# Levicoz/Options-model

Hardware: AMD Instinct MI355X
Metric: paths x steps / sec (whole American pricing: path-gen + LSM + mean) (higher is better)
Workload: dtype f32

## Files before the change

### options_model_amd/_build.py

```python
from __future__ import annotations

import os
import shutil
import subprocess
import sys

_HERE = os.path.dirname(os.path.abspath(__file__))
CSRC = os.path.join(_HERE, "csrc")
LIBDIR = os.path.join(_HERE, "lib")
LIB = os.path.join(LIBDIR, "libomc.so")
SOURCES = ["omc_paths.hip", "omc_lsm.hip", "omc_batch.hip", "omc_mlp.hip", "omc_mlp_batch.hip", "omc_mlp_apply.hip", "omc_nn_epoch.hip", "omc_contnet.hip", "omc_rows.hip", "omc_ols7.hip", "omc_greeks.hip", "omc_barrier.hip", "omc_dividend.hip", "omc_jump.hip", "omc_basket.hip", "omc_bounds.hip", "omc_basket_bounds.hip", "omc_runnerup_bounds.hip", "omc_heston_bounds.hip", "omc_heston_sv_bounds.hip", "omc_basket_greeks.hip", "omc_chain.hip", "omc_comm.hip", "omc_p2p.hip",
           "omc_api.hip", "omc_api_price.hip", "omc_api_seq.hip", "omc_api_batch.hip", "omc_api_nn.hip",
           "omc_api_bounds.hip", "omc_api_chain.hip", "omc_api_dividend.hip", "omc_api_jump.hip", "omc_api_basket.hip",
           "omc_api_basket_bounds.hip", "omc_api_runnerup_bounds.hip", "omc_api_basket_greeks.hip",
           "omc_api_heston_bounds.hip"]
HEADERS = ["omc_ctx.h", "omc_device.h", "omc_dispatch.h", "omc_crit.h", "omc_kernels.h", "omc_lsm_dev.h", "omc_paths_dev.h", "omc_contnet_dev.h", "omc_mlp_dev.h", "omc_mlp_quad_dev.h", "omc_batch.h", "omc_greeks.h", "omc_barrier.h", "omc_dividend.h", "omc_jump.h", "omc_basket.h", "omc_basket_dev.h", "omc_bounds.h", "omc_bounds_dev.h", "omc_bounds2_dev.h", "omc_basket_bounds.h", "omc_runnerup_bounds.h", "omc_heston_bounds.h", "omc_heston_sv_bounds.h", "omc_basket_greeks.h", "omc_chain.h", "omc_comm.h", "omc_p2p.h",
           os.path.join("..", "..", "include", "omc.h")]
ARCH = "gfx950"
FLAGS_STAMP = os.path.join(LIBDIR, "libomc.flags")


def _flags() -> str:
    return " ".join(os.environ.get("OMC_HIPCC_FLAGS", "").split())


def _hipcc() -> str:
    for cand in (os.environ.get("HIPCC"), shutil.which("hipcc"), "/opt/rocm/bin/hipcc"):
        if cand and os.path.exists(cand):
            return cand
    raise RuntimeError("hipcc not found: libomc.so cannot be built (ROCm toolchain required)")


def _stale() -> bool:
    if not os.path.exists(LIB):
        return True
    try:
        built_with = open(FLAGS_STAMP).read().strip()
    except OSError:
        built_with = ""
    if built_with != _flags():
        return True
    t = os.path.getmtime(LIB)
    deps = [os.path.join(CSRC, s) for s in SOURCES + HEADERS] + [os.path.abspath(__file__)]
    return any(os.path.getmtime(d) > t for d in deps)


def build(force: bool = False, verbose: bool = False) -> str:
    if not force and not _stale():
        return LIB
# ... 32 lines not shown
```

### options_model_amd/csrc/omc_api.hip

```cpp
#include <sched.h>

#include "omc_ctx.h"

namespace omc::abi {

thread_local std::string g_err;
size_t g_alloc_limit = 0;

int check_market(double S0, double K, double T, double r)
{
    if (!(S0 > 0) || !(K > 0) || !(T > 0)) return fail(-1, "S0, K, T must be positive.");
    if (!(r >= 0)) return fail(-2, "r must be non-negative.");
    return 0;
}

int check_sizes(int64_t n_paths, int n_steps)
{
    if (n_paths <= 0 || n_steps <= 0)
        return fail(-3, "num_simulations and num_time_steps must be positive integers.");
    if (n_steps > omc::kMaxSteps) return fail(-8, "num_time_steps exceeds the supported maximum (4094).");
    return 0;
}

int check_matrix(const void* S, int64_t ld, int64_t n_paths)
// ... 679 lines not shown
    int rc = bind_in(c);
    if (rc) return rc;
    if (!bytes) return 0;
    HIP_TRY(hipMemcpyAsync(dst, src, bytes, kind, c->stream));
    HIP_TRY(hipStreamSynchronize(c->stream));
    return 0;
}

int omc_memcpy_h2d(omc_ctx* c, void* dst, const void* src, size_t bytes)
{
    return copy_and_wait(c, dst, src, bytes, hipMemcpyHostToDevice);
}

int omc_memcpy_d2h(omc_ctx* c, void* dst, const void* src, size_t bytes)
{
    return copy_and_wait(c, dst, src, bytes, hipMemcpyDeviceToHost);
}

int omc_set_option(omc_ctx* c, const char* key, int64_t value)
{
    if (!c || !key) return fail(-7, "null pointer.");
    if (!strcmp(key, "gbm_vec")) c->gbm_vec = (int)value;
    else if (!strcmp(key, "alloc_limit")) g_alloc_limit = value > 0 ? (size_t)value : 0;
    else if (!strcmp(key, "fold_antithetic")) c->fold = value <= 0 ? 0 : (value >= 2 ? 2 : 1);
    else if (!strcmp(key, "pass2_tables")) c->pass2_tables = value ? 1 : 0;
    else if (!strcmp(key, "pass2_tables_irregular_every")) c->pass2_irr_every = value > 0 ? (int)value : 0;
    else if (!strcmp(key, "heston_vec")) c->heston_vec = (int)value;
    else if (!strcmp(key, "world_size")) c->world = value > 0 ? (int)value : 1;
    else if (!strcmp(key, "step_graph")) c->step_graph = value < 0 ? -1 : (value ? 1 : 0);
    else if (!strcmp(key, "seq_overlap")) c->seq_overlap = value < 0 ? -1 : (value ? 1 : 0);
    else if (!strcmp(key, "seq_event_stride")) c->seq_event_stride = value > 0 ? (int)value : 0;
    else if (!strcmp(key, "seq_step_k")) c->seq_step_k = value < 0 ? -1 : (int)(value > 32 ? 32 : value);
    else if (!strcmp(key, "seq_two_pass_k")) c->seq_two_pass_k = value < 0 ? -1 : (int)(value > 32 ? 32 : value);
    else if (!strcmp(key, "chain_fused")) c->chain_fused = value ? 1 : 0;
    else if (!strcmp(key, "chain_k")) c->chain_k = value < 1 ? -1 : (int)(value > 16 ? 16 : value);
    else if (!strcmp(key, "seq_step_wgs")) c->seq_step_wgs = value > 0 ? (int)value : 0;
    else if (!strcmp(key, "p2p_exchange")) c->p2p_use = value ? 1 : 0;
    else if (!strcmp(key, "p2p_deadline_ms") || !strcmp(key, "p2p_first_deadline_ms")) {
        if (value <= 0) return fail(-4, "a p2p deadline must be positive.");
        (key[4] == 'f' ? c->p2p_first_deadline_s : c->p2p_deadline_s) = (double)value * 1e-3;
        if (c->p2p) omc::p2p_set_deadline(c->p2p, c->p2p_deadline_s, c->p2p_first_deadline_s);
    }
    else return fail(-4, "unknown option key.");
    return 0;
}

int omc_set_allreduce_hook(omc_ctx* c, omc_allreduce_fn fn, void* user)
{
    if (!c) return fail(-7, "null context.");
    if (fn) {
        int rc;
        if ((rc = bind(c))) return rc;
        if ((rc = c->seq_vote.ensure(kVoteBytes))) return rc;
    }
    c->hook = fn;
    c->hook_user = user;
    return 0;
}

int omc_comm_unique_id(void* uid_out, size_t bytes)
{
    if (!uid_out || bytes < (size_t)omc::kCommUidBytes) return fail(-7, "unique-id buffer must hold 128 bytes.");
    std::string err;
    const int rc = omc::comm_unique_id(uid_out, &err);
    if (rc) return fail(rc, err.c_str());
    return 0;
// ... 116 lines not shown
```

### options_model_amd/csrc/omc_api_seq.hip

```cpp
#include <cstdlib>

#include "omc_ctx.h"

using namespace omc::abi;

extern "C" {

static int pricing_events(omc_ctx* c, int i, hipEvent_t** out)
{
    const int k = c->seq_event_stride, s = i == 0 ? 0 : (k > 0 && i % k == 0) ? i / k : -1;
    *out = s == 0 ? c->ev : nullptr;
    if (s <= 0) return 0;
    while (c->ev_pool.size() < 7 * (size_t)s) {
        hipEvent_t e = nullptr;
        HIP_TRY(hipEventCreate(&e));
        c->ev_pool.push_back(e);
    }
    *out = c->ev_pool.data() + 7 * (size_t)(s - 1);
    return 0;
}

static bool seq_overlap_enabled(const omc_ctx* c)
{
    if (c->seq_overlap >= 0) return c->seq_overlap != 0;
// ... 295 lines not shown
            q.T != p[0].T)
            break;
        double c0q, gq;
        omc::gbm_fold_constants(q.S0, q.K, q.r, q.sigma, q.T, q.n_steps, &c0q, &gq);
        if (c0q != c0 || gq != g) break;
    }
    return run;
}

static size_t seq_group_matrix_bytes(const omc_params* p)
{
    return sizeof(float) * (size_t)padded_ld(p->n_paths / 2) * ((size_t)p->n_steps + 1);
}

static int seq_group_ideal(const omc_ctx* c, const omc_params* p, int run)
{
    if (run < 2) return 1;
    static const int env_k = getenv("OMC_SEQ_TWO_PASS_K") ? atoi(getenv("OMC_SEQ_TWO_PASS_K")) : -1;
    int k = c->seq_two_pass_k >= 0 ? c->seq_two_pass_k : env_k;
    if (k < 0) k = (double)p[0].n_paths * (double)p[0].n_steps > 536870912.0 ? 1 : 8;
    if (k > omc::kSeqGroupMax) k = omc::kSeqGroupMax;
    if (k > run) k = run;
    return k < 2 ? 1 : k;
}

static int seq_group_fit(const omc_ctx* c, const omc_params* p, int k)
{
    const GroupLayout L(p[0].n_paths, p[0].n_steps);
    const int fit = (int)(seq_resident_budget(c, c->gS.cap + c->gstate.cap) / ((double)seq_group_matrix_bytes(p) + (double)L.per));
    if (k > fit) k = fit;
    return k < 2 ? 1 : k;
}

static int seq_group_reserve(omc_ctx* c, const omc_params* p, int run, int* K_out)
{
    *K_out = 1;
    int K = seq_group_ideal(c, p, run);
    const GroupLayout L(p[0].n_paths, p[0].n_steps);
    const size_t sbytes = seq_group_matrix_bytes(p);
    if (K >= 2 && (c->gS.cap < sbytes * (size_t)K || c->gstate.cap < L.per * (size_t)K)) K = seq_group_fit(c, p, K);
    while (K >= 2) {
        int rc = c->gS.ensure(sbytes * (size_t)K);
        if (!rc) rc = c->gstate.ensure(L.per * (size_t)K);
        if (!rc) break;
        if (rc != (int)hipErrorOutOfMemory && rc != (int)hipErrorMemoryAllocation) return rc;
        K /= 2;
    }
    *K_out = K < 2 ? 1 : K;
    return 0;
}

static int enqueue_seq_group(omc_ctx* c, const omc_params* p, int i0, int Kb, double* dst)
{
    int rc;
    const int64_t M = p[i0].n_paths;
    const int N = p[i0].n_steps;
    const size_t sbytes = seq_group_matrix_bytes(&p[i0]);
    int64_t ld = 0;
    const double* cK = nullptr;
    if ((rc = plan_storage(c, &p[i0], 0, &ld, &cK))) return rc;
    omc::LsmWorkspace w0;
    if ((rc = prepare_lsm(c, M, N, p[i0].r, p[i0].T, true, false, &w0))) return rc;
    if (!cK || ld != padded_ld(M / 2) || Kb > omc::kSeqGroupMax) return fail(-4, "a grouped two-pass sequence needs folded storage.");
    TwoPassGroup grp(GroupLayout(M, N), c->gstate.p, w0, true);
    hipEvent_t* evs[omc::kSeqGroupMax];
    for (int k = 0; k < Kb; ++k) {
        hipEvent_t* grown = nullptr;
        if ((rc = pricing_events(c, i0 + k, &grown))) return rc;
    }
    for (int k = 0; k < Kb; ++k) {
        const omc_params& q = p[i0 + k];
        float* S = (float*)((char*)c->gS.p + sbytes * (size_t)k);
        omc::LsmProblem prob{S, ld, M, N, q.is_put ? 1 : 0, q.K, q.r, q.T};
        prob.fold_cK = cK;
        grp.add(prob, dst + 8 * (size_t)(i0 + k));
        if ((rc = pricing_events(c, i0 + k, &evs[k]))) return rc;
        if (evs[k]) {
            grp.w[k].ev_p1_end = evs[k][4]; grp.w[k].ev_p2_end = evs[k][6];
            HIP_TRY(hipEventRecord(evs[k][0], c->stream));
        }
        if ((rc = enqueue_paths(c, &q, S, ld, true))) return rc;
        if (evs[k]) HIP_TRY(hipEventRecord(evs[k][1], c->stream));
        HIP_TRY(omc::lsm_pass1_sweep(c->stream, prob, grp.w[k], &grp.g.ntiles));
    }
    HIP_TRY(grp.reduce_pass1(c->stream));
    HIP_TRY(grp.build_tables(c->stream));
    for (int k = 0; k < Kb; ++k) {
        if (evs[k]) HIP_TRY(hipEventRecord(evs[k][5], c->stream));
        HIP_TRY(omc::lsm_pass2_sweep(c->stream, grp.prob[k], grp.w[k], false, true, &grp.g.nblk));
    }
    HIP_TRY(grp.finalize(c->stream));
    if (i0 == 0) HIP_TRY(hipEventRecord(c->ev[2], c->stream));
    return 0;
}

int omc_seq_group_width(omc_ctx* c, const omc_params* p, int n)
{
    if (!c || !p || n <= 0) return 0;
    for (int i = 0; i < n; ++i)
        if (check_params(&p[i])) return 0;
    const int run = seq_group_run(c, p, n);
    const int k = seq_group_ideal(c, p, run);
    return k < 2 ? 1 : seq_group_fit(c, p, k);
}

int omc_price_american_seq(omc_ctx* c, const omc_params* p, int n, omc_result* res)
{
    int rc;
    if ((rc = bind(c))) return rc;
    if (!p || !res || n <= 0) return fail(-7, "null pointer or empty sequence.");
    for (int i = 0; i < n; ++i)
        if ((rc = check_params(&p[i]))) return rc;
    if (!c->hres_dev) {
        for (int i = 0; i < n; ++i)
            if ((rc = omc_price_american(c, &p[i], &res[i], nullptr, 0))) return rc;
        return 0;
    }
    if (c->seq_cap < n) {
        if (c->seq_pin) (void)hipHostFree(c->seq_pin);
        c->seq_pin = c->seq_dev = nullptr;
        c->seq_cap = 0;
        HIP_TRY(hipHostMalloc((void**)&c->seq_pin, sizeof(double) * 8 * (size_t)n, hipHostMallocMapped));
        HIP_TRY(hipHostGetDevicePointer((void**)&c->seq_dev, c->seq_pin, 0));
        c->seq_cap = n;
    }
    hipEvent_t ev_end = c->ev[2];
    if (!c->ev_seq) HIP_TRY(hipEventCreate(&c->ev_seq));
    ev_end = c->ev_seq;
    const bool overlapped = seq_can_overlap(c, p, n);
    int multi = 1;
    if (!overlapped && (rc = seq_multi_reserve(c, p, n, &multi))) return rc;
    if (overlapped && (rc = enqueue_seq_overlapped(c, p, n, c->seq_pin))) return rc;
    const bool dist = c->distributed() && !overlapped;
    if (dist && (rc = c->seq_local.ensure(sizeof(double) * 8 * (size_t)n))) return rc;
    double* local = (double*)c->seq_local.p;
    c->defer_result_allreduce = dist;
    if (multi > 1 && (rc = enqueue_seq_step_multi(c, p, n, multi, dist ? local : c->seq_dev))) {
        c->defer_result_allreduce = false;
        return rc;
    }
    for (int i = 0; i < n && !overlapped && multi <= 1;) {
        int run = seq_group_run(c, &p[i], n - i), Kg = 1;
        if (run >= 2 && (rc = seq_group_reserve(c, &p[i], run, &Kg))) break;
        while (Kg >= 2 && run >= 2 && !rc) {
            const int Kb = Kg < run ? Kg : run;
            rc = enqueue_seq_group(c, p, i, Kb, c->seq_dev);
            i += Kb;
            run -= Kb;
        }
        for (; run >= 1 && !rc; ++i, --run) {
            hipEvent_t* evs = nullptr;
            if ((rc = pricing_events(c, i, &evs))) break;
            rc = enqueue_pricing(c, &p[i], nullptr, 0, dist ? local + 8 * (size_t)i : c->seq_dev + 8 * (size_t)i,
                                 evs, nullptr);
            if (!rc && evs && i == 0 && hipEventRecord(evs[2], c->stream) != hipSuccess) rc = fail(999, "hipEventRecord failed");
        }
        if (rc) break;
    }
    c->defer_result_allreduce = false;
    if (rc) return rc;
    if (dist) {
        if (c->p2p_used) HIP_TRY(omc::p2p_stamp_results(c->p2p, c->stream, local, n));
        if ((rc = allreduce(c, local, 8 * n))) return rc;
        HIP_TRY(hipMemcpyAsync(c->seq_pin, local, sizeof(double) * 8 * (size_t)n, hipMemcpyDeviceToHost, c->stream));
    }
    HIP_TRY(hipEventRecord(ev_end, c->stream));
    if ((rc = wait_stream(c))) return rc;
    if ((rc = check_p2p(c, c->seq_pin, n))) return rc;
    float ms_all = 0;
    HIP_TRY(hipEventElapsedTime(&ms_all, c->ev[0], ev_end));
    omc_result timed;
    memset(&timed, 0, sizeof timed);
    for (int i = 0; i < n; ++i) {
        hipEvent_t* evs = nullptr;
        if ((multi <= 1 || i == 0) && (rc = pricing_events(c, i, &evs))) return rc;
        if (evs) {
// ... 18 lines not shown
```

### options_model_amd/csrc/omc_ctx.h

```cpp
#pragma once
#include <hip/hip_runtime.h>

#include <cmath>
#include <cstdio>
#include <cstring>
#include <functional>
#include <string>
#include <vector>

#include "../../include/omc.h"
#include "omc_basket.h"
#include "omc_bounds.h"
#include "omc_comm.h"
#include "omc_kernels.h"
#include "omc_p2p.h"

namespace omc::abi {

extern thread_local std::string g_err;

inline int fail(int code, const char* msg)
{
    g_err = msg;
    return code;
// ... 169 lines not shown
    bool own_stream = false;
    DevBuf S, sx, tex, ex, D, part, gmom, betas, part1, result, scratch, sweep_args, crit;
    DevBuf bslab, btable, bres, bdisc;
    DevBuf mlp_part, mlp_loss, mlp_wt;
    DevBuf mlp_gred, shard;
    DevBuf cn_scratch, cn_data, cn_net, cn_cont;
    std::vector<char> h_table;
    std::vector<double> h_disc, h_bres;
    std::vector<double> hD;
    int D_N = -1;
    double D_r = 0, D_T = 0;
    const double* D_ptr = nullptr;
    double hres[8];
    double* hres_pin = nullptr;
    double* hres_dev = nullptr;
    double *seq_pin = nullptr, *seq_dev = nullptr;
    int seq_cap = 0;
    hipEvent_t ev_seq = nullptr;
    hipEvent_t ev_entry = nullptr;
    hipEvent_t ev[7] = {nullptr, nullptr, nullptr, nullptr, nullptr, nullptr, nullptr};
    std::vector<hipEvent_t> ev_pool;
    int seq_event_stride = 0;
    DevBuf mS, mstate, mtable;
    DevBuf mb_slab, mb_table, mb_bc;
    std::vector<double> mb_bc_host;
    double mb_beta1 = -1.0, mb_beta2 = -1.0;
    size_t mb_bc_cap = 0;
    char* mtab_pin = nullptr;
    int mtab_slot = 0;
    int seq_step_k = -1;
    int seq_step_wgs = 0;
    DevBuf gS, gstate;
    int seq_two_pass_k = -1;
    int gbm_vec = 0, heston_vec = 0;
    int fold = 1;
    int pass2_tables = 1;
    int pass2_irr_every = 0;
    DevBuf foldC;
    DevBuf gk_part, gk_res;
    DevBuf bar_part, bar_res;
    DevBuf div_tab;
    DevBuf bnd;
    DevBuf chain_fold;
    int chain_fused = 0;
    int chain_k = -1;
    struct FoldKey { int N = -1; double c0 = 0, g = 0; } fold_key[2];
    int world = 1;
    omc_allreduce_fn hook = nullptr;
    void* hook_user = nullptr;
    omc::Comm* comm = nullptr;
    omc::P2P* p2p = nullptr;
    int p2p_use = 1;
    bool p2p_used = false;
    double p2p_deadline_s = 2.0;
    double p2p_first_deadline_s = 30.0;
    hipStream_t comm_stream = nullptr;
    hipEvent_t ev_moments[2] = {nullptr, nullptr}, ev_reduced[2] = {nullptr, nullptr};
    RowsCache rows_cache;
    DevBuf S2, seq_local, part1b, gmomb, seq_vote;
    int seq_overlap = -1;
    bool defer_result_allreduce = false;
    hipGraph_t sweep_graph = nullptr;
    hipGraphExec_t sweep_exec = nullptr;
    int64_t sg_M = -1, sg_ld = -1;
    int sg_N = -1, sg_sem = -1, sg_vec4 = -1, sg_failed = 0;
    const void* sg_args = nullptr;
// ... 10 lines not shown
```

### options_model_amd/csrc/omc_kernels.h

```cpp
#pragma once
#include <hip/hip_runtime.h>
#include <stdint.h>

#include <atomic>
#include <cmath>

#include "omc_dispatch.h"

namespace omc {

inline hipError_t set_max_dynamic_lds(std::atomic<uint64_t>& mask, const void* kernel, size_t bytes)
{
    int dev = 0;
    hipError_t e = hipGetDevice(&dev);
    if (e != hipSuccess) return e;
    const uint64_t bit = 1ull << (dev & 63);
    if (mask.load(std::memory_order_acquire) & bit) return hipSuccess;
    e = hipFuncSetAttribute(kernel, hipFuncAttributeMaxDynamicSharedMemorySize, (int)bytes);
    if (e != hipSuccess) return e;
    mask.fetch_or(bit, std::memory_order_release);
    return hipSuccess;
}

struct PathSpec {
// ... 110 lines not shown
                        int nblk, int N);

hipError_t lsm_step(hipStream_t st, const LsmProblem& p, const LsmWorkspace& w, int semantics,
                    int t, bool external_moments);
hipError_t lsm_reduce_step_moments(hipStream_t st, const LsmWorkspace& w, int t, int nblk);
int lsm_step_blocks(int64_t M);
int lsm_sweep_blocks(int64_t M);
constexpr int kStepThreads = 1024;
template <class F>
inline void for_step(int semantics, bool v4, F&& f)
{
    for_int<0, 1>(semantics, [&](auto sem) {
        for_vec4(v4, [&](auto vec) { f(sem, vec, std::integral_constant<int, kStepThreads>{}); });
    });
}
size_t lsm_sweep_args_bytes();
void lsm_sweep_args_image(const LsmProblem& p, const LsmWorkspace& w, int semantics, bool fill_state, void* out,
                          bool external_moments = false);
int lsm_multi_groups(int64_t M, int K, int device_cus);
hipError_t lsm_step_multi(hipStream_t st, const void* table_dev, int K, int G, int semantics, bool vec4, int N, int t);
hipError_t lsm_reduce_step_moments_multi(hipStream_t st, const void* table_dev, int K, int t);
hipError_t lsm_final_multi(hipStream_t st, const void* table_dev, int K, int64_t M);
hipError_t lsm_sweep_indirect(hipStream_t st, const LsmProblem& p, const LsmWorkspace& w, int semantics,
                              const void* args_dev);

hipError_t lsm_pass1_moments(hipStream_t st, const LsmProblem& p, const LsmWorkspace& w);
hipError_t lsm_pass2_apply(hipStream_t st, const LsmProblem& p, const LsmWorkspace& w,
                           bool write_state, bool solve_from_moments = false);
hipError_t lsm_pass1_sweep(hipStream_t st, const LsmProblem& p, const LsmWorkspace& w, int64_t* ntiles);
hipError_t lsm_reduce_pass1(hipStream_t st, const LsmWorkspace& w, int64_t ntiles, int N);
bool lsm_pass2_tables(const LsmProblem& p, const LsmWorkspace& w, bool write_state);
hipError_t lsm_pass2_sweep(hipStream_t st, const LsmProblem& p, const LsmWorkspace& w, bool write_state,
                           bool solve_from_moments, int* nblk);
constexpr int kPass1Tpw = 4, kFoldTpw = 2;
struct Pass1Geometry {
    bool v4 = false;
    int tchunk = 32;
    int64_t ntiles = 0;
    dim3 grid;
};
Pass1Geometry lsm_pass1_geometry(const LsmProblem& p);
struct FoldGeometry {
    Pass1Geometry p1;
    int fvec = 2, vec2 = 1, nblk = 0;
};
FoldGeometry lsm_fold_geometry(const LsmProblem& p);
constexpr int kSeqGroupMax = 32;
struct SeqGroupSlot {
    const double* part1;
    double* gmom;
    double* betas;
    uint32_t* crit;
    const double* part;
    double* result;
    const double* cK;
    double K, invK;
    int is_put, pad_;
};
struct SeqGroupArgs {
    SeqGroupSlot slot[kSeqGroupMax];
    int64_t ntiles;
    int N, nblk;
    int irr_every, pad_;
};
static_assert(sizeof(SeqGroupSlot) == 80 && sizeof(SeqGroupArgs) == 80 * kSeqGroupMax + 24 && sizeof(SeqGroupArgs) <= 4096,
              "the group's argument block travels by value in the kernel arguments");
// ... 126 lines not shown
```

### options_model_amd/csrc/omc_lsm.hip

```cpp
#include "omc_lsm_dev.h"

#include <cstdlib>
#include <cstring>

namespace omc {

template <int SEM, int VEC, int BLOCK>
__global__ __launch_bounds__(BLOCK) void lsm_step_kernel(StepArgs a)
{
    lsm_step_body<SEM, VEC, BLOCK>(a, blockIdx.x, a.nblk);
}

template <int SEM, int VEC, int BLOCK>
__global__ __launch_bounds__(BLOCK) void lsm_step_ind_kernel(const StepArgs* __restrict__ ap, int t)
{
    StepArgs a = *ap;
    a.t = t;
    lsm_step_body<SEM, VEC, BLOCK>(a, blockIdx.x, a.nblk);
}

__global__ __launch_bounds__(kBlock) void lsm_reduce_step_kernel(const double* part, double* gmom, int t,
                                                                 int nblk, int pstride, int gstride)
{
    lsm_reduce_step_body(part, gmom, t, nblk, pstride, gstride);
}

template <int VEC, int TPW, int PUT>
__global__ __launch_bounds__(kBlock) void lsm_pass1_kernel(Pass1Args a) { lsm_pass1_body<VEC, TPW, PUT>(a); }

__global__ __launch_bounds__(kBlock) void lsm_reduce_pass1_kernel(const double* part1, double* gmom,
                                                                  int64_t ntiles, int N)
{
    lsm_reduce_pass1_body(part1, gmom, ntiles, N);
}

__global__ void lsm_solve_betas_kernel(const double* __restrict__ gmom, double* __restrict__ betas, int N)
{
    lsm_solve_all_body(gmom, betas, N);
}

template <int VEC, bool WRITE_STATE>
__global__ __launch_bounds__(kBlock) void lsm_pass2_kernel(Pass2Args a) { lsm_pass2_body<VEC, WRITE_STATE>(a); }

template <int VEC, int TPW, int PUT>
__global__ __launch_bounds__(kBlock) void lsm_pass1_fold_kernel(Pass1Args a) { lsm_pass1_fold_body<VEC, TPW, PUT>(a); }
template <int VEC, int PUT, bool TAB>
__global__ __launch_bounds__(kBlock) void lsm_pass2_fold_kernel(Pass2Args a) { lsm_pass2_fold_body<VEC, PUT, TAB>(a); }

__global__ __launch_bounds__(128) void lsm_crit_build_kernel(CritArgs a) { lsm_crit_build_body(a); }
__global__ __launch_bounds__(kBlock) void lsm_crit_check_kernel(const uint32_t* tab, const double* betas, const double* cK,
                                                                int N, int is_put, double K, double invK,
                                                                unsigned long long* mism)
{
    lsm_crit_check_body(tab, betas, cK, N, is_put, K, invK, mism);
}

__global__ void lsm_fold_table_kernel(double* __restrict__ cK, int N, double c0, double g)
{
    if (threadIdx.x == 0 && blockIdx.x == 0) fold_table_fill(cK, N, c0, g);
}

template <int VEC>
__global__ __launch_bounds__(kBlock) void lsm_final_kernel(FinalArgs a) { lsm_final_body<VEC>(a); }

template <int VEC>
__global__ __launch_bounds__(kBlock) void lsm_final_ind_kernel(const FinalArgs* __restrict__ ap)
{
    lsm_final_body<VEC>(*ap);
}

__global__ __launch_bounds__(kBlock) void lsm_finalize_kernel(const double* part, const double* gmom,
                                                              double* result, int nblk, int N, int pstride)
{
    lsm_finalize_body(part, gmom, result, nblk, N, pstride);
}

struct FinalizeArgs {
    const double* part;
    const double* gmom;
    double* result;
// ... 336 lines not shown
    const int nblk = fold ? geo.nblk : lsm_step_blocks(p.M);
    *nblk_out = nblk;
    if (fold && write_state) return hipErrorInvalidValue;
    Pass2Args a = pass2_args(p, w, nblk);
    const bool tab = lsm_pass2_tables(p, w, write_state);
    if (tab) {
        a.crit = w.crit;
    } else if (solve_from_moments) {
        a.gmom = w.gmom;
        a.betas_out = w.betas;
    }
    const size_t dyn = sizeof(double) * 4 * (size_t)(p.N + 1);
    const dim3 grid(nblk), block(kBlock);
    if (fold) {
        for_vec(geo.vec2, [&](auto vec) {
            for_put(p.is_put, [&](auto put) {
                for_flag(tab, [&](auto tb) {
                    constexpr int VEC = decltype(vec)::value, PUT = decltype(put)::value;
                    hipLaunchKernelGGL((lsm_pass2_fold_kernel<VEC, PUT, decltype(tb)::value>), grid, block, dyn, st, a);
                });
            });
        });
    } else {
        for_vec4(rows_aligned(4, p.M, p.S, p.ld), [&](auto vec) {
            for_flag(write_state, [&](auto ws) {
                hipLaunchKernelGGL((lsm_pass2_kernel<decltype(vec)::value, decltype(ws)::value>), grid, block, dyn, st, a);
            });
        });
    }
    if (w.ev_p2_end) (void)hipEventRecord(w.ev_p2_end, st);
    return hipGetLastError();
}

hipError_t lsm_pass2_apply(hipStream_t st, const LsmProblem& p, const LsmWorkspace& w,
                           bool write_state, bool solve_from_moments)
{
    if (w.ev_p2_begin) (void)hipEventRecord(w.ev_p2_begin, st);
    const bool tab = lsm_pass2_tables(p, w, write_state);
    if (tab) {
        CritArgs c;
        c.gmom = solve_from_moments ? w.gmom : nullptr; c.betas = w.betas; c.betas_out = solve_from_moments ? w.betas : nullptr;
        c.cK = p.fold_cK; c.tab = w.crit;
        c.N = p.N; c.is_put = p.is_put; c.K = p.K; c.irr_every = w.crit_irr_every;
        const hipError_t e = lsm_crit_build(st, c);
        if (e != hipSuccess) return e;
    }
    int nblk = 0;
    const hipError_t e = lsm_pass2_sweep(st, p, w, write_state, solve_from_moments, &nblk);
    return e != hipSuccess ? e : lsm_finalize(st, w.part, w.gmom, w.result, nblk, p.N);
}

SeqGroupSlot lsm_group_slot(const LsmProblem& p, const LsmWorkspace& w)
{
    SeqGroupSlot s;
    s.part1 = w.part1; s.gmom = w.gmom; s.betas = w.betas; s.crit = w.crit; s.part = w.part; s.result = w.result;
    s.cK = p.fold_cK;
    s.K = p.K; s.invK = 1.0 / p.K; s.is_put = p.is_put; s.pad_ = 0;
    return s;
}

hipError_t lsm_group_reduce_pass1(hipStream_t st, const SeqGroupArgs& g, int K)
{
    if (g.N < 2) return hipSuccess;
    hipLaunchKernelGGL(lsm_reduce_pass1_group_kernel, dim3(g.N - 1, K), dim3(kBlock), 0, st, g);
    return hipGetLastError();
}
// ... 59 lines not shown
```

### options_model_amd/csrc/omc_lsm_dev.h

```cpp
#pragma once
#include "omc_device.h"
#include "omc_kernels.h"
#include "omc_crit.h"
#include <type_traits>

namespace omc {


constexpr int kPStride = kMaxLsmBlocks;

template <int VEC>
__device__ __forceinline__ void loadf(const float* __restrict__ p, float (&v)[VEC])
{
    if constexpr (VEC == 4) {
        const float4 x = *reinterpret_cast<const float4*>(p);
        v[0] = x.x; v[1] = x.y; v[2] = x.z; v[3] = x.w;
    } else if constexpr (VEC == 2) {
        const float2 x = *reinterpret_cast<const float2*>(p);
        v[0] = x.x; v[1] = x.y;
    } else {
        static_assert(VEC == 1, "loadf: 1, 2 or 4 floats");
        v[0] = *p;
    }
}
template <int VEC>
__device__ __forceinline__ void loadf_stream(const float* __restrict__ p, float (&v)[VEC])
{
    if constexpr (VEC == 4) {
        typedef float f4 __attribute__((ext_vector_type(4)));
        const f4 x = __builtin_nontemporal_load(reinterpret_cast<const f4*>(p));
        v[0] = x.x; v[1] = x.y; v[2] = x.z; v[3] = x.w;
    } else if constexpr (VEC == 2) {
        typedef float f2 __attribute__((ext_vector_type(2)));
        const f2 x = __builtin_nontemporal_load(reinterpret_cast<const f2*>(p));
        v[0] = x.x; v[1] = x.y;
    } else {
// ... 435 lines not shown
                load_rows(bufB, min(t + 4, tl));
                __builtin_amdgcn_sched_barrier(0);
                process(put_tag, bufC, t + 2);
            }
        }
    };
    if (PUT == 1 || (PUT < 0 && is_put))
        sweep(std::true_type{});
    else
        sweep(std::false_type{});
}

__device__ __forceinline__ double fold_rcp(float s)
{
    const double x = (double)s;
    double r = __builtin_amdgcn_rcp(x);
    r = fma(fma(-x, r, 1.0), r, r);
    return r;
}
__device__ __forceinline__ double fold_u_rcp(double cK_t, double rcp_s) { return fma(cK_t, rcp_s, -1.0); }
__device__ __forceinline__ double fold_u(double cK_t, float s) { return fold_u_rcp(cK_t, fold_rcp(s)); }
__device__ __forceinline__ double fold_pay(double u, double K, int is_put) { return is_put ? -K * u : K * u; }
__device__ __forceinline__ void fold_table_fill(double* __restrict__ tab, int N, double c0, double g)
{
    double c = c0;
    tab[0] = c;
    for (int t = 1; t <= N; ++t) {
        c *= g;
        tab[t] = c;
    }
}
constexpr int kFoldMaxChunk = 64;

template <int VEC, int TPW, int PUT = -1>
__device__ __forceinline__ void lsm_pass1_fold_body(Pass1Args a)
{
    __shared__ double wl[kBlock / 64][kWaveRedDoubles];
    __shared__ double shD[kBlock / 64][kFoldMaxChunk];
    __shared__ double shC[kBlock / 64][kFoldMaxChunk];
    const int lane = threadIdx.x & 63, wave = threadIdx.x >> 6;
    const int64_t tg = (int64_t)xcd_block((int)blockIdx.x, (int)gridDim.x) * (kBlock / 64) + wave;
    if (tg >= a.ntiles) return;
    const int64_t base = tg * (64 * VEC * TPW) + (int64_t)lane * VEC;
    const int t0 = 1 + ((int)gridDim.y - 1 - (int)blockIdx.y) * a.tchunk;
    const int t1 = min(t0 + a.tchunk, a.N);
    if (t0 >= t1) return;
    const double K = a.K, invK = a.invK;
    const int is_put = PUT < 0 ? a.is_put : PUT;
    for (int i = lane; i < t1 - t0; i += 64) {
        shD[wave][i] = a.D[a.N - (t0 + i)];
        shC[wave][i] = a.cK[t0 + i];
    }
    const float* colp[TPW];
    double pNA[TPW][VEC], pNB[TPW][VEC];
    bool valid[TPW];
    const double cKN = a.cK[a.N];
    float sn[TPW][VEC];
#pragma unroll
    for (int k = 0; k < TPW; ++k) {
        const int64_t j = base + (int64_t)k * 64 * VEC;
        valid[k] = j < a.M;
        colp[k] = a.S + (valid[k] ? j : 0);
        loadf<VEC>(colp[k] + (int64_t)a.N * a.ld, sn[k]);
    }
    auto load_rows = [&](float (&buf)[TPW][VEC], int t) {
#pragma unroll
        for (int k = 0; k < TPW; ++k) loadf_stream<VEC>(colp[k] + (int64_t)t * a.ld, buf[k]);
    };
    float bufA[TPW][VEC], bufB[TPW][VEC], bufC[TPW][VEC];
    const int tl = t1 - 1;
    load_rows(bufA, t0);
    load_rows(bufB, min(t0 + 1, tl));
    __builtin_amdgcn_sched_barrier(0);
#pragma unroll
    for (int k = 0; k < TPW; ++k) {
#pragma unroll
        for (int v = 0; v < VEC; ++v) {
// ... 394 lines not shown
        auto live = [&]() {
            bool l = false;
#pragma unroll
            for (int v = 0; v < VEC; ++v) l |= (tex[v] == N);
            return l;
        };
        constexpr int U = 8;
        int t = N - 1;
        const float* col = a.S + j;
        for (; t >= U && live(); t -= U) {
            float st[U][VEC];
#pragma unroll
            for (int k = 0; k < U; ++k) loadf_stream<VEC>(col + (int64_t)(t - k) * a.ld, st[k]);
#pragma unroll
            for (int k = 0; k < U; ++k) decide(st[k], t - k);
        }
        for (; t >= 1 && live(); --t) {
            float st[VEC];
            loadf_stream<VEC>(col + (int64_t)t * a.ld, st);
            decide(st, t);
        }
#pragma unroll
        for (int v = 0; v < VEC; ++v) add_cash_flow(acc, payoff_d(sx[v], K, is_put), a.D[tex[v] - 1], tex[v] < N);
        if (WRITE_STATE) {
            storef<VEC>(a.sx + j, sx);
            storei<VEC>(a.tex + j, tex);
        }
    }
    const double s = block_reduce8(acc, red);
    if (tid < 64 && (tid & 7) == 0) a.part[(size_t)(tid >> 3) * a.pstride + blockIdx.x] = s;
}

template <int VEC, int PUT = -1, bool TAB = false>
__device__ __forceinline__ void lsm_pass2_fold_body(Pass2Args a)
{
    if ((int)blockIdx.x >= a.nblk) return;
    __shared__ double red[kNQ * kRedStride];
    extern __shared__ double sh_b[];
    uint32_t* sh_t = reinterpret_cast<uint32_t*>(sh_b);
    const int tid = threadIdx.x;
    const int N = a.N;
    bool irr_any = false;
    if (TAB) irr_any = crit_load_tables(a.crit, sh_t, N);
    else fits_to_lds<true>(sh_b, a.gmom, a.betas_out, a.betas, a.cK, N);
    const double K = a.K, invK = a.invK;
    const int is_put = PUT < 0 ? a.is_put : PUT;
    double acc[8];
#pragma unroll
    for (int q = 0; q < 8; ++q) acc[q] = 0.0;
    const int64_t stride = (int64_t)a.nblk * kBlock * VEC;
    auto sweep = [&](auto chk) {
    constexpr bool CHK = decltype(chk)::value;
    for (int64_t j = ((int64_t)blockIdx.x * kBlock + tid) * VEC; j < a.M; j += stride) {
        float sxa[VEC], sxb[VEC];
        int32_t texa[VEC], texb[VEC];
        loadf<VEC>(a.S + (int64_t)N * a.ld + j, sxa);
#pragma unroll
        for (int v = 0; v < VEC; ++v) {
            sxb[v] = sxa[v];
            texa[v] = texb[v] = N;
        }
        auto decide_f64 = [&](const float (&row)[VEC], int t, const Fit& f, double ck) {
#pragma unroll
            for (int v = 0; v < VEC; ++v) {
                const bool ex = (texa[v] == N) & exercises(pay_stored(row[v], K, invK, is_put), f);
                sxa[v] = ex ? row[v] : sxa[v];
                texa[v] = ex ? t : texa[v];
                const bool exb = (texb[v] == N) & exercises(pay_partner(ck, row[v], K, is_put), f);
                sxb[v] = exb ? row[v] : sxb[v];
                texb[v] = exb ? t : texb[v];
            }
        };
        auto decide = [&](const float (&row)[VEC], int t) {
            if constexpr (!TAB) {
                decide_f64(row, t, fit_lds(sh_b, t), sh_b[4 * t + 3]);
            } else {
                const uint4 ta = *reinterpret_cast<const uint4*>(sh_t + 8 * t);
                if (CHK && __builtin_amdgcn_readfirstlane(ta.x) == kCritIrregular) {
                    decide_f64(row, t, fit_given(a.betas, t, N), a.cK[t]);
                    return;
                }
                const uint4 tb = *reinterpret_cast<const uint4*>(sh_t + 8 * t + 4);
#pragma unroll
                for (int v = 0; v < VEC; ++v) {
                    const uint32_t bits = __float_as_uint(row[v]);
                    const bool ex = (texa[v] == N) & crit_in(ta, bits);
                    sxa[v] = ex ? row[v] : sxa[v];
                    texa[v] = ex ? t : texa[v];
                    const bool exb = (texb[v] == N) & crit_in(tb, bits);
                    sxb[v] = exb ? row[v] : sxb[v];
                    texb[v] = exb ? t : texb[v];
                }
            }
        };
        auto live = [&]() {
            bool l = false;
#pragma unroll
            for (int v = 0; v < VEC; ++v) l |= (texa[v] == N) | (texb[v] == N);
            return l;
        };
        walk_rows<VEC, TAB>(a.S + j, a.ld, N, decide, live);
#pragma unroll
        for (int v = 0; v < VEC; ++v) {
            add_cash_flow(acc, payoff_d(sxa[v], K, is_put), a.D[texa[v] - 1], texa[v] < N);
            const double ck = TAB ? a.cK[texb[v]] : sh_b[4 * texb[v] + 3];
            add_cash_flow(acc, pay_partner(ck, sxb[v], K, is_put).imm, a.D[texb[v] - 1], texb[v] < N);
        }
    }
    };
    if (TAB && irr_any) sweep(std::true_type{});
    else sweep(std::false_type{});
    const double s = block_reduce8(acc, red);
    if (tid < 64 && (tid & 7) == 0) a.part[(size_t)(tid >> 3) * a.pstride + blockIdx.x] = s;
}

struct FinalArgs {
    float* sx;
    int32_t* tex;
    const float* live;
    int64_t M;
    int N, is_put, tval, fill_state;
    double K;
    const double* D;
    double* part;
    int nblk, pstride;
};

template <int VEC>
__device__ __forceinline__ void lsm_final_body(FinalArgs a)
{
    if ((int)blockIdx.x >= a.nblk) return;
    __shared__ double red[kNQ * kRedStride];
    const int tid = threadIdx.x;
    double acc[8];
#pragma unroll
    for (int q = 0; q < 8; ++q) acc[q] = 0.0;
    const int64_t stride = (int64_t)a.nblk * kBlock * VEC;
    for (int64_t j = ((int64_t)blockIdx.x * kBlock + tid) * VEC; j < a.M; j += stride) {
        float sx[VEC];
        int32_t tex[VEC];
        loadf<VEC>(a.sx + j, sx);
        loadi<VEC>(a.tex + j, tex);
        if (a.live) {
            float sn[VEC];
            loadf<VEC>(a.live + j, sn);
            bool any = false;
#pragma unroll
// ... 42 lines not shown
```

Measured before the change: 771.4 billion.

## Fuse pass1 of one group with pass2 of previous group in a paired sweep kernel

```diff
diff --git a/options_model_amd/_build.py b/options_model_amd/_build.py
--- a/options_model_amd/_build.py
+++ b/options_model_amd/_build.py
@@ -14,7 +14,7 @@
            "omc_api_bounds.hip", "omc_api_chain.hip", "omc_api_dividend.hip", "omc_api_jump.hip", "omc_api_basket.hip",
            "omc_api_basket_bounds.hip", "omc_api_runnerup_bounds.hip", "omc_api_basket_greeks.hip",
            "omc_api_heston_bounds.hip"]
-HEADERS = ["omc_ctx.h", "omc_device.h", "omc_dispatch.h", "omc_crit.h", "omc_kernels.h", "omc_lsm_dev.h", "omc_paths_dev.h", "omc_contnet_dev.h", "omc_mlp_dev.h", "omc_mlp_quad_dev.h", "omc_batch.h", "omc_greeks.h", "omc_barrier.h", "omc_dividend.h", "omc_jump.h", "omc_basket.h", "omc_basket_dev.h", "omc_bounds.h", "omc_bounds_dev.h", "omc_bounds2_dev.h", "omc_basket_bounds.h", "omc_runnerup_bounds.h", "omc_heston_bounds.h", "omc_heston_sv_bounds.h", "omc_basket_greeks.h", "omc_chain.h", "omc_comm.h", "omc_p2p.h",
+HEADERS = ["omc_ctx.h", "omc_device.h", "omc_dispatch.h", "omc_crit.h", "omc_pair_map.h", "omc_kernels.h", "omc_lsm_dev.h", "omc_paths_dev.h", "omc_contnet_dev.h", "omc_mlp_dev.h", "omc_mlp_quad_dev.h", "omc_batch.h", "omc_greeks.h", "omc_barrier.h", "omc_dividend.h", "omc_jump.h", "omc_basket.h", "omc_basket_dev.h", "omc_bounds.h", "omc_bounds_dev.h", "omc_bounds2_dev.h", "omc_basket_bounds.h", "omc_runnerup_bounds.h", "omc_heston_bounds.h", "omc_heston_sv_bounds.h", "omc_basket_greeks.h", "omc_chain.h", "omc_comm.h", "omc_p2p.h",
            os.path.join("..", "..", "include", "omc.h")]
 ARCH = "gfx950"
 FLAGS_STAMP = os.path.join(LIBDIR, "libomc.flags")
diff --git a/options_model_amd/csrc/omc_api.hip b/options_model_amd/csrc/omc_api.hip
--- a/options_model_amd/csrc/omc_api.hip
+++ b/options_model_amd/csrc/omc_api.hip
@@ -735,6 +735,7 @@
     else if (!strcmp(key, "seq_event_stride")) c->seq_event_stride = value > 0 ? (int)value : 0;
     else if (!strcmp(key, "seq_step_k")) c->seq_step_k = value < 0 ? -1 : (int)(value > 32 ? 32 : value);
     else if (!strcmp(key, "seq_two_pass_k")) c->seq_two_pass_k = value < 0 ? -1 : (int)(value > 32 ? 32 : value);
+    else if (!strcmp(key, "seq_pair")) c->seq_pair = value < 0 ? -1 : (value ? 1 : 0);
     else if (!strcmp(key, "chain_fused")) c->chain_fused = value ? 1 : 0;
     else if (!strcmp(key, "chain_k")) c->chain_k = value < 1 ? -1 : (int)(value > 16 ? 16 : value);
     else if (!strcmp(key, "seq_step_wgs")) c->seq_step_wgs = value > 0 ? (int)value : 0;
diff --git a/options_model_amd/csrc/omc_api_seq.hip b/options_model_amd/csrc/omc_api_seq.hip
--- a/options_model_amd/csrc/omc_api_seq.hip
+++ b/options_model_amd/csrc/omc_api_seq.hip
@@ -351,21 +351,37 @@
     return k < 2 ? 1 : k;
 }
 
-static int seq_group_reserve(omc_ctx* c, const omc_params* p, int run, int* K_out)
+static bool seq_pair_wanted(const omc_ctx* c, const omc_params* p)
+{
+    if (c->seq_pair >= 0) return c->seq_pair != 0;
+    static const int env = getenv("OMC_SEQ_PAIR") ? atoi(getenv("OMC_SEQ_PAIR")) : -1;
+    if (env >= 0) return env != 0;
+    return (double)p[0].n_paths * (double)p[0].n_steps <= 167772160.0;
+}
+
+static int seq_group_reserve(omc_ctx* c, const omc_params* p, int run, int* K_out, bool* pair)
 {
     *K_out = 1;
+    *pair = false;
     int K = seq_group_ideal(c, p, run);
+    int sets = K >= 2 && run >= K + 2 && seq_pair_wanted(c, p) ? 2 : 1;
     const GroupLayout L(p[0].n_paths, p[0].n_steps);
     const size_t sbytes = seq_group_matrix_bytes(p);
-    if (K >= 2 && (c->gS.cap < sbytes * (size_t)K || c->gstate.cap < L.per * (size_t)K)) K = seq_group_fit(c, p, K);
+    if (K >= 2 && (c->gS.cap < sbytes * (size_t)(K * sets) || c->gstate.cap < L.per * (size_t)(K * sets))) {
+        const int fit = seq_group_fit(c, p, K * sets);
+        if (fit < K * sets) sets = 1;
+        if (fit < K) K = fit;
+    }
     while (K >= 2) {
-        int rc = c->gS.ensure(sbytes * (size_t)K);
-        if (!rc) rc = c->gstate.ensure(L.per * (size_t)K);
+        int rc = c->gS.ensure(sbytes * (size_t)(K * sets));
+        if (!rc) rc = c->gstate.ensure(L.per * (size_t)(K * sets));
         if (!rc) break;
         if (rc != (int)hipErrorOutOfMemory && rc != (int)hipErrorMemoryAllocation) return rc;
-        K /= 2;
+        if (sets == 2) sets = 1;
+        else K /= 2;
     }
     *K_out = K < 2 ? 1 : K;
+    *pair = K >= 2 && sets == 2;
     return 0;
 }
 
@@ -413,6 +429,72 @@
     return 0;
 }
 
+static int enqueue_seq_groups_paired(omc_ctx* c, const omc_params* p, int i0, int n, int K, double* dst)
+{
+    int rc;
+    const int64_t M = p[i0].n_paths;
+    const int N = p[i0].n_steps;
+    const size_t sbytes = seq_group_matrix_bytes(&p[i0]);
+    int64_t ld = 0;
+    const double* cK = nullptr;
+    if ((rc = plan_storage(c, &p[i0], 0, &ld, &cK))) return rc;
+    omc::LsmWorkspace w0;
+    if ((rc = prepare_lsm(c, M, N, p[i0].r, p[i0].T, true, false, &w0))) return rc;
+    if (!cK || ld != padded_ld(M / 2) || K > omc::kSeqGroupMax) return fail(-4, "a grouped two-pass sequence needs folded storage.");
+    const GroupLayout L(M, N);
+    for (int i = 0; i < n; ++i) {
+        hipEvent_t* grown = nullptr;
+        if ((rc = pricing_events(c, i0 + i, &grown))) return rc;
+    }
+    TwoPassGroup grp[2] = {TwoPassGroup(L, c->gstate.p, w0, true), TwoPassGroup(L, (char*)c->gstate.p + L.per * (size_t)K, w0, true)};
+    hipEvent_t* evs[2][omc::kSeqGroupMax];
+    const int G = (n + K - 1) / K;
+    int Kprev = 0;
+    for (int g = 0; g <= G; ++g) {
+        const int s = g & 1, Kb = g == G ? 0 : (n - g * K < K ? n - g * K : K);
+        TwoPassGroup &cur = grp[s], &prev = grp[s ^ 1];
+        if (Kb) cur = TwoPassGroup(L, (char*)c->gstate.p + L.per * (size_t)(K * s), w0, true);
+        for (int k = 0; k < (Kb > Kprev ? Kb : Kprev); ++k) {
+            const bool has1 = k < Kb, has2 = k < Kprev;
+            if (has1) {
+                const int i = i0 + g * K + k;
+                float* S = (float*)((char*)c->gS.p + sbytes * (size_t)(K * s + k));
+                omc::LsmProblem prob{S, ld, M, N, p[i].is_put ? 1 : 0, p[i].K, p[i].r, p[i].T};
+                prob.fold_cK = cK;
+                cur.add(prob, dst + 8 * (size_t)i);
+                if ((rc = pricing_events(c, i, &evs[s][k]))) return rc;
+                if (evs[s][k]) {
+                    cur.w[k].ev_p1_end = evs[s][k][4]; cur.w[k].ev_p2_end = evs[s][k][6];
+                    HIP_TRY(hipEventRecord(evs[s][k][0], c->stream));
+                }
+                if ((rc = enqueue_paths(c, &p[i], S, ld, true))) return rc;
+                if (evs[s][k]) HIP_TRY(hipEventRecord(evs[s][k][1], c->stream));
+            }
+            if (has1 && has2 && !evs[s][k] && !evs[s ^ 1][k]) {
+                bool paired = false;
+                HIP_TRY(omc::lsm_sweep_pair(c->stream, cur.prob[k], cur.w[k], prev.prob[k], prev.w[k], &cur.g.ntiles,
+                                            &prev.g.nblk, &paired));
+                continue;
+            }
+            if (has1) HIP_TRY(omc::lsm_pass1_sweep(c->stream, cur.prob[k], cur.w[k], &cur.g.ntiles));
+            if (has2) {
+                if (evs[s ^ 1][k]) HIP_TRY(hipEventRecord(evs[s ^ 1][k][5], c->stream));
+                HIP_TRY(omc::lsm_pass2_sweep(c->stream, prev.prob[k], prev.w[k], false, true, &prev.g.nblk));
+            }
+        }
+        if (Kprev) {
+            HIP_TRY(prev.finalize(c->stream));
+            if (i0 == 0 && g == 1) HIP_TRY(hipEventRecord(c->ev[2], c->stream));
+        }
+        if (Kb) {
+            HIP_TRY(cur.reduce_pass1(c->stream));
+            HIP_TRY(cur.build_tables(c->stream));
+        }
+        Kprev = Kb;
+    }
+    return 0;
+}
+
 int omc_seq_group_width(omc_ctx* c, const omc_params* p, int n)
 {
     if (!c || !p || n <= 0) return 0;
@@ -460,7 +542,14 @@
     }
     for (int i = 0; i < n && !overlapped && multi <= 1;) {
         int run = seq_group_run(c, &p[i], n - i), Kg = 1;
-        if (run >= 2 && (rc = seq_group_reserve(c, &p[i], run, &Kg))) break;
+        bool pair = false;
+        if (run >= 2 && (rc = seq_group_reserve(c, &p[i], run, &Kg, &pair))) break;
+        if (pair) {
+            const int m = run % Kg == 1 ? run - 1 : run;
+            rc = enqueue_seq_groups_paired(c, p, i, m, Kg, c->seq_dev);
+            i += m;
+            run -= m;
+        }
         while (Kg >= 2 && run >= 2 && !rc) {
             const int Kb = Kg < run ? Kg : run;
             rc = enqueue_seq_group(c, p, i, Kb, c->seq_dev);
diff --git a/options_model_amd/csrc/omc_ctx.h b/options_model_amd/csrc/omc_ctx.h
--- a/options_model_amd/csrc/omc_ctx.h
+++ b/options_model_amd/csrc/omc_ctx.h
@@ -225,6 +225,7 @@
     int seq_step_wgs = 0;
     DevBuf gS, gstate;
     int seq_two_pass_k = -1;
+    int seq_pair = -1;
     int gbm_vec = 0, heston_vec = 0;
     int fold = 1;
     int pass2_tables = 1;
diff --git a/options_model_amd/csrc/omc_kernels.h b/options_model_amd/csrc/omc_kernels.h
--- a/options_model_amd/csrc/omc_kernels.h
+++ b/options_model_amd/csrc/omc_kernels.h
@@ -166,6 +166,8 @@
 bool lsm_pass2_tables(const LsmProblem& p, const LsmWorkspace& w, bool write_state);
 hipError_t lsm_pass2_sweep(hipStream_t st, const LsmProblem& p, const LsmWorkspace& w, bool write_state,
                            bool solve_from_moments, int* nblk);
+hipError_t lsm_sweep_pair(hipStream_t st, const LsmProblem& p1, const LsmWorkspace& w1, const LsmProblem& p2,
+                          const LsmWorkspace& w2, int64_t* ntiles, int* nblk, bool* paired);
 constexpr int kPass1Tpw = 4, kFoldTpw = 2;
 struct Pass1Geometry {
     bool v4 = false;
diff --git a/options_model_amd/csrc/omc_lsm.hip b/options_model_amd/csrc/omc_lsm.hip
--- a/options_model_amd/csrc/omc_lsm.hip
+++ b/options_model_amd/csrc/omc_lsm.hip
@@ -1,5 +1,6 @@
 #include "omc_lsm_dev.h"
 
+#include <cstdio>
 #include <cstdlib>
 #include <cstring>
 
@@ -43,9 +44,33 @@
 __global__ __launch_bounds__(kBlock) void lsm_pass2_kernel(Pass2Args a) { lsm_pass2_body<VEC, WRITE_STATE>(a); }
 
 template <int VEC, int TPW, int PUT>
-__global__ __launch_bounds__(kBlock) void lsm_pass1_fold_kernel(Pass1Args a) { lsm_pass1_fold_body<VEC, TPW, PUT>(a); }
+__global__ __launch_bounds__(kBlock) void lsm_pass1_fold_kernel(Pass1Args a)
+{
+    __shared__ Pass1FoldLds lds;
+    lsm_pass1_fold_body<VEC, TPW, PUT>(a, lds, make_int2((int)blockIdx.x, (int)blockIdx.y), make_int2((int)gridDim.x, (int)gridDim.y));
+}
 template <int VEC, int PUT, bool TAB>
-__global__ __launch_bounds__(kBlock) void lsm_pass2_fold_kernel(Pass2Args a) { lsm_pass2_fold_body<VEC, PUT, TAB>(a); }
+__global__ __launch_bounds__(kBlock) void lsm_pass2_fold_kernel(Pass2Args a)
+{
+    __shared__ double red[kNQ * kRedStride];
+    extern __shared__ double sh_b[];
+    lsm_pass2_fold_body<VEC, PUT, TAB>(a, red, sh_b, blockIdx.x);
+}
+
+template <int PUT1, int PUT2>
+__global__ __launch_bounds__(kBlock) void lsm_sweep_pair_kernel(Pass1Args a1, Pass2Args a2, SweepPairMap m)
+{
+    extern __shared__ __attribute__((aligned(16))) double pair_lds[];
+    int v = 0;
+    const int role = m.role((int)blockIdx.x, &v);
+    if (role == 1) {
+        const int by = v / m.g1x;
+        lsm_pass1_fold_body<4, kFoldTpw, PUT1>(a1, *reinterpret_cast<Pass1FoldLds*>(pair_lds), make_int2(v - by * m.g1x, by),
+                                               make_int2(m.g1x, m.g1y));
+    } else if (role == 2) {
+        lsm_pass2_fold_body<2, PUT2, true>(a2, pair_lds, pair_lds + kNQ * kRedStride, (unsigned)v);
+    }
+}
 
 __global__ __launch_bounds__(128) void lsm_crit_build_kernel(CritArgs a) { lsm_crit_build_body(a); }
 __global__ __launch_bounds__(kBlock) void lsm_crit_check_kernel(const uint32_t* tab, const double* betas, const double* cK,
@@ -448,6 +473,55 @@
     return hipGetLastError();
 }
 
+static void pair_pattern(int* a, int* b)
+{
+    static const int env = [] {
+        const char* e = getenv("OMC_SEQ_PAIR_PATTERN");
+        int x = -1, y = -1;
+        if (!e || sscanf(e, "%d:%d", &x, &y) != 2 || x < 0 || y < 0 || x > 255 || y > 255 || (x == 0) != (y == 0)) return -1;
+        return x * 256 + y;
+    }();
+    *a = env < 0 ? 2 : env / 256;
+    *b = env < 0 ? 1 : env % 256;
+}
+
+hipError_t lsm_sweep_pair(hipStream_t st, const LsmProblem& p1, const LsmWorkspace& w1, const LsmProblem& p2,
+                          const LsmWorkspace& w2, int64_t* ntiles, int* nblk, bool* paired)
+{
+    *paired = false;
+    const size_t dyn2 = kPairRedBytes + sizeof(uint32_t) * 8 * (size_t)(p2.N + 1);
+    const size_t dyn = dyn2 > sizeof(Pass1FoldLds) ? dyn2 : sizeof(Pass1FoldLds);
+    bool can = p1.fold_cK && p2.fold_cK && p1.N >= 2 && lsm_pass2_tables(p2, w2, false) && dyn <= 40960 &&
+               !w1.ev_p1_begin && !w1.ev_p1_end && !w2.ev_p2_end;
+    FoldGeometry g1, g2;
+    if (can) {
+        g1 = lsm_fold_geometry(p1);
+        g2 = lsm_fold_geometry(p2);
+        can = g1.p1.v4 && g2.vec2 == 2 && (int64_t)g1.p1.grid.x * g1.p1.grid.y + g2.nblk < (int64_t(1) << 30);
+    }
+    if (!can) {
+        const hipError_t e = lsm_pass1_sweep(st, p1, w1, ntiles);
+        return e != hipSuccess ? e : lsm_pass2_sweep(st, p2, w2, false, true, nblk);
+    }
+    const Pass1Args a1 = pass1_args(p1, w1, g1.p1.ntiles, g1.p1.tchunk);
+    Pass2Args a2 = pass2_args(p2, w2, g2.nblk);
+    a2.crit = w2.crit;
+    int pa = 0, pb = 0;
+    pair_pattern(&pa, &pb);
+    const SweepPairMap m = sweep_pair_map((int)g1.p1.grid.x, (int)g1.p1.grid.y, g2.nblk, pa, pb);
+    const dim3 grid((unsigned)m.blocks());
+    for_put(p1.is_put, [&](auto put1) {
+        for_put(p2.is_put, [&](auto put2) {
+            hipLaunchKernelGGL((lsm_sweep_pair_kernel<decltype(put1)::value, decltype(put2)::value>), grid, dim3(kBlock), dyn, st,
+                               a1, a2, m);
+        });
+    });
+    *ntiles = a1.ntiles;
+    *nblk = g2.nblk;
+    *paired = true;
+    return hipGetLastError();
+}
+
 hipError_t lsm_pass2_apply(hipStream_t st, const LsmProblem& p, const LsmWorkspace& w,
                            bool write_state, bool solve_from_moments)
 {
diff --git a/options_model_amd/csrc/omc_lsm_dev.h b/options_model_amd/csrc/omc_lsm_dev.h
--- a/options_model_amd/csrc/omc_lsm_dev.h
+++ b/options_model_amd/csrc/omc_lsm_dev.h
@@ -2,6 +2,7 @@
 #include "omc_device.h"
 #include "omc_kernels.h"
 #include "omc_crit.h"
+#include "omc_pair_map.h"
 #include <type_traits>
 
 namespace omc {
@@ -503,17 +504,22 @@
 }
 constexpr int kFoldMaxChunk = 64;
 
+struct Pass1FoldLds {
+    double wl[kBlock / 64][kWaveRedDoubles];
+    double shC[kBlock / 64][kFoldMaxChunk];
+    double shD[kBlock / 64][kFoldMaxChunk];
+};
 template <int VEC, int TPW, int PUT = -1>
-__device__ __forceinline__ void lsm_pass1_fold_body(Pass1Args a)
-{
-    __shared__ double wl[kBlock / 64][kWaveRedDoubles];
-    __shared__ double shD[kBlock / 64][kFoldMaxChunk];
-    __shared__ double shC[kBlock / 64][kFoldMaxChunk];
+__device__ __forceinline__ void lsm_pass1_fold_body(Pass1Args a, Pass1FoldLds& lds, int2 blk, int2 grid)
+{
+    auto& wl = lds.wl;
+    auto& shD = lds.shD;
+    auto& shC = lds.shC;
     const int lane = threadIdx.x & 63, wave = threadIdx.x >> 6;
-    const int64_t tg = (int64_t)xcd_block((int)blockIdx.x, (int)gridDim.x) * (kBlock / 64) + wave;
+    const int64_t tg = (int64_t)xcd_block(blk.x, grid.x) * (kBlock / 64) + wave;
     if (tg >= a.ntiles) return;
     const int64_t base = tg * (64 * VEC * TPW) + (int64_t)lane * VEC;
-    const int t0 = 1 + ((int)gridDim.y - 1 - (int)blockIdx.y) * a.tchunk;
+    const int t0 = 1 + (grid.y - 1 - blk.y) * a.tchunk;
     const int t1 = min(t0 + a.tchunk, a.N);
     if (t0 >= t1) return;
     const double K = a.K, invK = a.invK;
@@ -974,11 +980,9 @@
 }
 
 template <int VEC, int PUT = -1, bool TAB = false>
-__device__ __forceinline__ void lsm_pass2_fold_body(Pass2Args a)
-{
-    if ((int)blockIdx.x >= a.nblk) return;
-    __shared__ double red[kNQ * kRedStride];
-    extern __shared__ double sh_b[];
+__device__ __forceinline__ void lsm_pass2_fold_body(Pass2Args a, double* red, double* sh_b, unsigned bx)
+{
+    if ((int)bx >= a.nblk) return;
     uint32_t* sh_t = reinterpret_cast<uint32_t*>(sh_b);
     const int tid = threadIdx.x;
     const int N = a.N;
@@ -993,7 +997,7 @@
     const int64_t stride = (int64_t)a.nblk * kBlock * VEC;
     auto sweep = [&](auto chk) {
     constexpr bool CHK = decltype(chk)::value;
-    for (int64_t j = ((int64_t)blockIdx.x * kBlock + tid) * VEC; j < a.M; j += stride) {
+    for (int64_t j = ((int64_t)bx * kBlock + tid) * VEC; j < a.M; j += stride) {
         float sxa[VEC], sxb[VEC];
         int32_t texa[VEC], texb[VEC];
         loadf<VEC>(a.S + (int64_t)N * a.ld + j, sxa);
@@ -1053,8 +1057,11 @@
     if (TAB && irr_any) sweep(std::true_type{});
     else sweep(std::false_type{});
     const double s = block_reduce8(acc, red);
-    if (tid < 64 && (tid & 7) == 0) a.part[(size_t)(tid >> 3) * a.pstride + blockIdx.x] = s;
-}
+    if (tid < 64 && (tid & 7) == 0) a.part[(size_t)(tid >> 3) * a.pstride + bx] = s;
+}
+
+constexpr size_t kPairRedBytes = sizeof(double) * kNQ * kRedStride;
+static_assert(kPairRedBytes % 16 == 0, "the tables behind the reduction rows are read 16 bytes at a time");
 
 struct FinalArgs {
     float* sx;
diff --git a/options_model_amd/csrc/omc_pair_map.h b/options_model_amd/csrc/omc_pair_map.h
--- /dev/null
+++ b/options_model_amd/csrc/omc_pair_map.h
@@ -0,0 +1,52 @@
+#pragma once
+
+#if defined(__HIPCC__)
+#define OMC_PAIR_HD __host__ __device__
+#else
+#define OMC_PAIR_HD
+#endif
+
+namespace omc {
+
+struct SweepPairMap {
+    int n1, n2, g1x, g1y;
+    int a, b, periods;
+    int units1, units2;
+    int blocks() const { return (units1 + units2) * 8; }
+    OMC_PAIR_HD int role(int bx, int* v) const
+    {
+        const int u = bx >> 3, r = bx & 7, ab = a + b;
+        int u1 = -1, u2 = -1;
+        if (u < periods * ab) {
+            const int p = u / ab, o = u - p * ab;
+            if (o < a) u1 = p * a + o;
+            else u2 = p * b + (o - a);
+        } else {
+            const int o = u - periods * ab, left1 = units1 - periods * a;
+            if (o < left1) u1 = periods * a + o;
+            else u2 = periods * b + (o - left1);
+        }
+        if (u1 >= 0) {
+            *v = u1 * 8 + r;
+            return *v < n1 ? 1 : 0;
+        }
+        *v = u2 * 8 + r;
+        return *v < n2 ? 2 : 0;
+    }
+};
+
+inline SweepPairMap sweep_pair_map(int g1x, int g1y, int n2, int a, int b)
+{
+    SweepPairMap m;
+    m.n1 = g1x * g1y; m.n2 = n2; m.g1x = g1x; m.g1y = g1y;
+    m.units1 = (m.n1 + 7) / 8;
+    m.units2 = (m.n2 + 7) / 8;
+    if (a < 1 || b < 1) { a = m.units1; b = m.units2; }
+    if (a < 1) a = 1;
+    if (b < 1) b = 1;
+    m.a = a; m.b = b;
+    m.periods = m.units1 / a < m.units2 / b ? m.units1 / a : m.units2 / b;
+    return m;
+}
+
+}
```

Measured after the change: 772.5 billion (median of 3 runs). No clear change (+0.2%).
